# IntelLabs/GKL

Hardware: AMD Instinct MI355X
Metric: pairhmm_gcups (higher is better)
Workload: dtype f32

## Files before the change

### gkl_amd/csrc/pairhmm_aux_kernels.h

```cpp
#pragma once
#include <hip/hip_runtime.h>
#include <stdint.h>

#include "../../include/gkl_hip_pairhmm.h"
#include "pairhmm_fwd_kernel.h"
#include "pairhmm_multi_sets.h"

namespace gklhip {

struct PrepArgs {
  const uint8_t* hap_bases;
  const int32_t* hap_src;
  const int32_t* hap_len;
  const int32_t* hap_pos;
  const int32_t* hap_group;
  const int32_t* hap_pos_flat;
  uint32_t* stream_flat;
  uint32_t* stream;
  uint8_t* hap_has_n;
  int32_t n_haps;
  int32_t* clear_a; int32_t n_a;
  int32_t* clear_b; int32_t n_b;
  int32_t* clear_c; int32_t n_c;
  const uint4* pull_src; uint4* pull_dst; int32_t pull_n16;
// ... 189 lines not shown
  int32_t* count;
  int32_t* read_fail;
  int32_t n_haps;
  int64_t n;
  int mode;
  float log10_init_f;
  double log10_init32_as_f64;
  double log10_init_d;
};

__global__ void finalize32_kernel(FinalizeArgs a) {
  const int64_t i = (int64_t)blockIdx.x * blockDim.x + threadIdx.x;
  if (i >= a.n || a.used64[i]) return;
  const float v = a.raw32[i];
  if (a.mode == GKLHIP_FINALIZE_DEVICE_F64) a.out[i] = log10((double)v) - a.log10_init32_as_f64;
  else if (a.mode == GKLHIP_FINALIZE_DEVICE_REF32) a.out[i] = (double)((float)log10((double)v) - a.log10_init_f);
}

__global__ void finalize64_kernel(FinalizeArgs a, int all_pairs) {
  const int64_t p = (int64_t)blockIdx.x * blockDim.x + threadIdx.x;
  if (p >= a.n) return;
  if (all_pairs) a.used64[p] = 1;
  else if (!a.used64[p]) return;
  if (a.mode >= 0) a.out[p] = log10(a.raw64[p]) - a.log10_init_d;
  if (a.mode == kModePacked) reinterpret_cast<uint64_t*>(a.out)[p] = packed_word(a.raw64[p]);
}

#ifndef GKL_PACK_WINDOW
#define GKL_PACK_WINDOW 96
#endif
constexpr int kPackWindow = GKL_PACK_WINDOW;
constexpr int kJobClasses = 64;
constexpr int kPlanBlock = 1024;

struct PlanArgs {
  FinalizeArgs fa;
  int32_t n_reads, n_haps, n_pairs_i;
  const int64_t* read_off;
  int32_t rpl;
  int32_t max_len;
  int32_t* cnts;
  int32_t* hist;
  int32_t* pos;
  int32_t* order;
  LaneSlot* lanes2;
  const int32_t* hap_orig;
  const int32_t* hap_group;
  const int32_t* hap_pos;
  const int32_t* hap_len;
  FwdJob* jobs;
  FwdJob* sorted;
  const LaneSlot* long_lanes;
  int32_t n_long;
  FwdJob* jobs_long;
  int32_t* long_chunk_jobs;
  int32_t total_cols;
  int32_t wanted_jobs;
  int32_t min_job_cols;
  int32_t packed_by_kernels;
};

__device__ __forceinline__ bool last_block_done(int32_t* arrivals) {
  __shared__ int32_t s_is_last;
  __syncthreads();
  if (threadIdx.x == 0) {
    __threadfence();
    const int32_t before = atomicAdd(arrivals, 1);
    s_is_last = before == (int32_t)gridDim.x - 1 ? 1 : 0;
    __threadfence();
  }
  __syncthreads();
  return s_is_last != 0;
}

__device__ __forceinline__ int32_t ld_cnt(int32_t* p) { return __hip_atomic_load(p, __ATOMIC_RELAXED, __HIP_MEMORY_SCOPE_AGENT); }

__device__ __forceinline__ int job_class(const FwdJob& j, const int32_t* hap_pos, const int32_t* hap_len) {
  const int cols = hap_pos[j.hap_end - 1] + hap_len[j.hap_end - 1] - hap_pos[j.hap_begin];
  const int c = cols >> 7;
  return kJobClasses - 1 - (c < kJobClasses - 1 ? c : kJobClasses - 1);
}

__device__ __forceinline__ void build_jobs_for_chunk(const PlanArgs& a, const LaneSlot* lanes, int c, FwdJob* jobs,
                                                     int32_t* chunk_jobs, int cut_cols, bool by_group, int lane) {
  const LaneSlot sl = lanes[(int64_t)c * kLanes + lane];
  jobs += (int64_t)c * a.n_haps;
  int n_jobs = 0;
  bool prev_need = false;
  uint64_t reads = __ballot(sl.read >= 0 && sl.block == 0);
  for (int k0 = 0; k0 < a.n_haps; k0 += kLanes) {
    const int k = k0 + lane;
    const bool in = k < a.n_haps;
    const int h = in ? a.hap_orig[k] : 0;
    uint8_t nd = 0;
    for (uint64_t m = reads; m; m &= m - 1) {
      const int r = __builtin_amdgcn_readlane(sl.read, __builtin_ctzll(m));
      if (in) nd |= a.fa.used64[(int64_t)r * a.n_haps + h];
    }
    const uint64_t need = __ballot(in && nd != 0);
    if (!need) { prev_need = false; continue; }
    bool start = false;
    if (in && nd) {
      const bool pred_needed = lane == 0 ? prev_need : ((need >> (lane - 1)) & 1ull) != 0;
      start = !pred_needed || a.hap_pos[k - 1] / cut_cols != a.hap_pos[k] / cut_cols ||
              (by_group && a.hap_group[k - 1] != a.hap_group[k]);
    }
    const uint64_t starts = __ballot(start);
    if ((need & 1ull) && !(starts & 1ull)) {
      const uint64_t stop = starts | ~need;
      const int e = stop ? __builtin_ctzll(stop) : kLanes;
      if (lane == 0) jobs[n_jobs - 1].hap_end = min(k0 + e, a.n_haps);
    }
    const int base = n_jobs;
    n_jobs += __builtin_popcountll(starts);
    if (start) {
      const uint64_t after = lane == kLanes - 1 ? 0ull : (~0ull << (lane + 1));
      const uint64_t stop = (starts | ~need) & after;
      const int e = stop ? __builtin_ctzll(stop) : kLanes;
      FwdJob j;
      j.chunk = c; j.hap_begin = k; j.hap_end = min(k0 + e, a.n_haps);
      j.klass = 0;
      jobs[base + __builtin_popcountll(starts & ((1ull << lane) - 1ull))] = j;
    }
    prev_need = ((need >> (kLanes - 1)) & 1ull) != 0;
  }
  __threadfence_block();
  for (int i = lane; i < n_jobs; i += kLanes) {
    FwdJob j = jobs[i];
    jobs[i].klass = job_class(j, a.hap_pos, a.hap_len);
  }
  if (lane == 0) chunk_jobs[c] = n_jobs;
}

#define GKLHIP_PLAN_STAMP(k) do { if (tid == 0) a.cnts[16 + (k)] = (int32_t)(wall_clock64() - clk0); } while (0)

constexpr int kPlanLdsBins = 4096;
template <bool kInLds>
__device__ __forceinline__ void order_affected_reads(const PlanArgs& a, int32_t* hist, int32_t* pos, int32_t* s_wave_tot,
                                                     int tid, uint64_t clk0) {
  constexpr int kBatch = 4;
  const int n = a.n_haps, lane = tid & 63, wave = tid >> 6;
  if (kInLds) {
    for (int c = tid; c < n + 2; c += kPlanBlock) hist[c] = 0;
    __syncthreads();
  }
  for (int r0 = tid; r0 < a.n_reads; r0 += kBatch * kPlanBlock) {
    int f[kBatch];
#pragma unroll
    for (int k = 0; k < kBatch; k++) {
      const int r = r0 + k * kPlanBlock;
      const bool in = r < a.n_reads;
      const int fr = in ? a.fa.read_fail[r] : 0;
      const int64_t len = in ? a.read_off[r + 1] - a.read_off[r] : 0;
      f[k] = (fr > 0 && len <= a.max_len) ? fr : 0;
    }
#pragma unroll
    for (int k = 0; k < kBatch; k++)
      if (f[k] > 0) atomicAdd(hist + f[k], 1);
  }
  __threadfence();
  __syncthreads();
  GKLHIP_PLAN_STAMP(0);

  {
    const int per = (n + kPlanBlock - 1) / kPlanBlock;
    const int hi = n - tid * per, lo = max(hi - per, 0);
    int sum = 0;
    for (int c = hi; c > lo; c--) sum += hist[c];
    int inc = sum;
    for (int d = 1; d < 64; d <<= 1) {
      const int o = __shfl_up(inc, d, 64);
      if (lane >= d) inc += o;
    }
    if (lane == 63) s_wave_tot[wave] = inc;
    __syncthreads();
    int base = 0, total = 0;
    for (int w = 0; w < kPlanBlock / 64; w++) {
      const int t = s_wave_tot[w];
      base += w < wave ? t : 0;
      total += t;
    }
    if (tid == 0) __hip_atomic_store(a.cnts + 4, total, __ATOMIC_RELAXED, __HIP_MEMORY_SCOPE_AGENT);
    int acc = base + inc - sum;
    for (int c = hi; c > lo; c--) { pos[c] = acc; acc += hist[c]; }
  }
  __threadfence();
  __syncthreads();
  GKLHIP_PLAN_STAMP(1);

  for (int r0 = tid; r0 < a.n_reads; r0 += kBatch * kPlanBlock) {
    int f[kBatch];
#pragma unroll
// ... 29 lines not shown
        const int leader = __builtin_ctzll(mask);
        const int32_t read = fails ? (int32_t)((uint32_t)i / (uint32_t)a.n_haps) : -1;
        const int32_t lead_read = __shfl(read, leader, 64);
        const uint64_t same = __ballot(fails && read == lead_read);
        if (lane == leader) atomicAdd(a.fa.read_fail + lead_read, __builtin_popcountll(same));
        if (fails && read != lead_read) atomicAdd(a.fa.read_fail + read, 1);
        if (lane == 0) my_fails += __builtin_popcountll(mask);
      }
      if (in_range) {
        a.fa.used64[i] = fails ? 1 : 0;
        if (a.fa.mode == kModePacked && !a.packed_by_kernels)
          reinterpret_cast<uint64_t*>(a.fa.out)[i] = fails ? 0ull : (kPackedF32Tag | (uint64_t)__float_as_uint(v));
      }
    }
    if (lane == 0) s_wave[wave] = my_fails;
    __syncthreads();
    if (tid == 0) {
      int total = 0;
      for (int w = 0; w < kPlanBlock / 64; w++) total += s_wave[w];
      if (total) atomicAdd(a.cnts + 0, total);
    }
  }
  if (!last_block_done(a.cnts + 10)) return;
  const int n_fail = ld_cnt(a.cnts + 0);
  if (n_fail == 0) return;
  const uint64_t clk0 = wall_clock64();

  if (a.n_haps + 2 <= kPlanLdsBins) order_affected_reads<true>(a, s_hist, s_hist + kPlanLdsBins, s_i32, tid, clk0);
  else                             order_affected_reads<false>(a, a.hist, a.pos, s_i32, tid, clk0);
  GKLHIP_PLAN_STAMP(2);
}

__global__ __launch_bounds__(kPlanBlock) void plan_pack_kernel(PlanArgs a) {
  const int tid = (int)threadIdx.x, lane = tid & 63, wave = tid >> 6;
  const int nblk = (int)gridDim.x, blk = (int)blockIdx.x;
  if (ld_cnt(a.cnts + 0) == 0) return;
  const uint64_t clk0 = wall_clock64();

  {
    static_assert(kPackWindow <= 2 * kLanes, "the window's lane counts sit in two registers per lane");
    __shared__ int32_t s_pack[kPlanBlock / 64][4][kPackWindow];
    int32_t* s_read = s_pack[wave][0]; int32_t* s_needl = s_pack[wave][1]; int32_t* s_sread = s_pack[wave][2];
    int32_t* s_sneed = s_pack[wave][3];
    const int n = ld_cnt(a.cnts + 4);
    const int n_win = (n + kPackWindow - 1) / kPackWindow;
    for (int w = blk * (kPlanBlock / 64) + wave; w < n_win; w += nblk * (kPlanBlock / 64)) {
      const int w0 = w * kPackWindow;
      const int cnt = min(kPackWindow, n - w0);
      for (int i = lane; i < cnt; i += kLanes) {
        const int r = a.order[w0 + i];
        s_read[i] = r;
        s_needl[i] = (int)((a.read_off[r + 1] - a.read_off[r] + a.rpl) / a.rpl);
      }
      __builtin_amdgcn_wave_barrier();
      if (w == 0 && lane == 0) a.cnts[22] = (int32_t)(wall_clock64() - clk0);
      for (int i = lane; i < cnt; i += kLanes) {
        const int ni = s_needl[i];
        int rank = 0;
        for (int j = 0; j < cnt; j++) {
          const int nj = s_needl[j];
          rank += (nj > ni) || (nj == ni && j < i);
        }
        s_sread[rank] = s_read[i];
        s_sneed[rank] = ni;
      }
      __builtin_amdgcn_wave_barrier();
      if (w == 0 && lane == 0) a.cnts[23] = (int32_t)(wall_clock64() - clk0);
      int head = -1, next_lo = -1, next_hi = -1;
      int bin_lo = 0, off_lo = 0, bin_hi = 0, off_hi = 0;
      uint64_t avail = 0;
      int nb = 0;
      const int need_lo = lane < cnt ? s_sneed[lane] : 0, need_hi = lane + kLanes < cnt ? s_sneed[lane + kLanes] : 0;
      for (int i = 0; i < cnt; i++) {
        const int nn = __builtin_amdgcn_readlane(i < kLanes ? need_lo : need_hi, i & 63);
        const uint64_t fits = nn >= kLanes ? 0ull : (avail >> nn) << nn;
        int bin, f;
        if (fits) {
          f = __builtin_ctzll(fits);
          bin = __builtin_amdgcn_readlane(head, f);
          const int nxt = __builtin_amdgcn_readlane(bin < kLanes ? next_lo : next_hi, bin & 63);
          if (lane == f) head = nxt;
          if (nxt < 0) avail &= ~(1ull << f);
        } else {
          bin = nb++;
          f = kLanes;
        }
        const int left = f - nn;
        if (left > 0) {
          const int old = __builtin_amdgcn_readlane(head, left);
          if (lane == (bin & 63)) { if (bin < kLanes) next_lo = old; else next_hi = old; }
          if (lane == left) head = bin;
          avail |= 1ull << left;
        }
        if (lane == (i & 63)) { if (i < kLanes) { bin_lo = bin; off_lo = kLanes - f; } else { bin_hi = bin; off_hi = kLanes - f; } }
      }
      if (w == 0 && lane == 0) a.cnts[24] = (int32_t)(wall_clock64() - clk0);
      int base = 0;
      if (lane == 0) base = atomicAdd(a.cnts + 5, nb);
      base = __shfl(base, 0, kLanes);
      LaneSlot idle; idle.read = -1; idle.block = 0;
      for (int i = lane; i < nb * kLanes; i += kLanes) a.lanes2[(int64_t)base * kLanes + i] = idle;
      __builtin_amdgcn_wave_barrier();
      __threadfence_block();
      if (w == 0 && lane == 0) a.cnts[25] = (int32_t)(wall_clock64() - clk0);
      if (lane < cnt) {
        LaneSlot sl; sl.read = s_sread[lane];
        LaneSlot* dst = a.lanes2 + (int64_t)(base + bin_lo) * kLanes + off_lo;
        for (int b = 0; b < need_lo; b++) { sl.block = b; dst[b] = sl; }
      }
      if (lane + kLanes < cnt) {
        LaneSlot sl; sl.read = s_sread[lane + kLanes];
        LaneSlot* dst = a.lanes2 + (int64_t)(base + bin_hi) * kLanes + off_hi;
        for (int b = 0; b < need_hi; b++) { sl.block = b; dst[b] = sl; }
      }
      __builtin_amdgcn_wave_barrier();
      if (w == 0 && lane == 0) a.cnts[26] = (int32_t)(wall_clock64() - clk0);
    }
  }
  if (blk == 0) GKLHIP_PLAN_STAMP(3);
}

__global__ __launch_bounds__(kPlanBlock) void plan_jobs_kernel(PlanArgs a) {
  __shared__ int32_t s_i32[kPlanBlock];
  const int tid = (int)threadIdx.x, lane = tid & 63, wave = tid >> 6;
  const int nblk = (int)gridDim.x, blk = (int)blockIdx.x;
  const int n_fail = ld_cnt(a.cnts + 0);
  if (n_fail == 0) return;
  const uint64_t clk0 = wall_clock64();

  {
    const int total = ld_cnt(a.cnts + 5);
    const int n_fail_reads = ld_cnt(a.cnts + 4);
    const double density = (double)n_fail / ((double)max(n_fail_reads, 1) * (double)a.n_haps);
    const double est_steps = (double)max(total, 1) * (double)a.total_cols * fmin(density, 1.0);
    const int cut_cols = max(a.min_job_cols, (int)fmin(est_steps / (double)a.wanted_jobs, 1e9));
    const int n_waves = nblk * (kPlanBlock / 64), w = blk * (kPlanBlock / 64) + wave;
    for (int c = w; c < total; c += n_waves) build_jobs_for_chunk(a, a.lanes2, c, a.jobs, a.order, cut_cols, false, lane);
    for (int c = w; c < a.n_long; c += n_waves) build_jobs_for_chunk(a, a.long_lanes, c, a.jobs_long, a.long_chunk_jobs, 0x7fffffff, true, lane);
  }
  if (!last_block_done(a.cnts + 11)) return;
  GKLHIP_PLAN_STAMP(4);

  {
    int32_t* cnt = s_i32;
    int32_t* base = s_i32 + kJobClasses;
    const int total = ld_cnt(a.cnts + 5);
    __syncthreads();
    if (tid < kJobClasses) cnt[tid] = 0;
    __syncthreads();
    for (int c = tid; c < total; c += kPlanBlock) {
      const FwdJob* mine = a.jobs + (int64_t)c * a.n_haps;
      const int n = a.order[c];
      for (int i = 0; i < n; i++) atomicAdd(&cnt[mine[i].klass], 1);
    }
    __syncthreads();
    if (tid == 0) {
      int acc = 0;
      for (int c = 0; c < kJobClasses; c++) { base[c] = acc; acc += cnt[c]; }
      a.cnts[2] = acc;
    }
    __syncthreads();
    for (int c = tid; c < total; c += kPlanBlock) {
      const FwdJob* mine = a.jobs + (int64_t)c * a.n_haps;
      const int n = a.order[c];
      for (int i = 0; i < n; i++) {
        const FwdJob j = mine[i];
        a.sorted[atomicAdd(&base[j.klass], 1)] = j;
      }
    }
    if (tid == 0 && a.n_long > 0) {
      int at = 0;
      for (int c = 0; c < a.n_long; c++) {
        const int n = a.long_chunk_jobs[c];
        for (int i = 0; i < n; i++) a.jobs_long[at++] = a.jobs_long[(int64_t)c * a.n_haps + i];
      }
      a.cnts[8] = at;
    }
  }
  GKLHIP_PLAN_STAMP(5);
}
#undef GKLHIP_PLAN_STAMP

__global__ void flush_selftest_kernel(uint32_t* out, float f, double d) {
  float fm;
  double dm;
  asm volatile("v_mul_f32 %0, 1.0, %1" : "=v"(fm) : "v"(f));
  asm volatile("v_mul_f64 %0, 1.0, %1" : "=v"(dm) : "v"(d));
  out[0] = __float_as_uint(fm);
  out[1] = (uint32_t)((uint64_t)__double_as_longlong(dm) >> 32) | (uint32_t)(uint64_t)__double_as_longlong(dm);
}

__global__ __launch_bounds__(256) void lds_oob_selftest_kernel(uint32_t* out) {
  __shared__ __attribute__((aligned(16))) uint32_t lds[4 * 2560];
  for (int i = threadIdx.x; i < 4 * 2560; i += 256) lds[i] = 0xA5A50000u | (uint32_t)i;
  __syncthreads();
  const uint32_t loff = (uint32_t)(uintptr_t)lds + (threadIdx.x >> 6) * 10240u + (threadIdx.x & 63u) * 16u;
  uint32_t acc = 0;
#pragma unroll
  for (int shift = 9; shift <= 11; shift++) {
    const uint32_t addr = (512u << shift) + loff;
    uint32_t v0, v1, v2, v3, w0, w1, w2, w3, x0, x1;
    asm volatile("ds_read_b128 v[40:43], %10\n\tds_read_b128 v[44:47], %10 offset:1024\n\tds_read_b64 v[48:49], %10\n\ts_waitcnt lgkmcnt(0)\n\t"
                 "v_mov_b32 %0, v40\n\tv_mov_b32 %1, v41\n\tv_mov_b32 %2, v42\n\tv_mov_b32 %3, v43\n\t"
                 "v_mov_b32 %4, v44\n\tv_mov_b32 %5, v45\n\tv_mov_b32 %6, v46\n\tv_mov_b32 %7, v47\n\tv_mov_b32 %8, v48\n\tv_mov_b32 %9, v49"
                 : "=v"(v0), "=v"(v1), "=v"(v2), "=v"(v3), "=v"(w0), "=v"(w1), "=v"(w2), "=v"(w3), "=v"(x0), "=v"(x1)
                 : "v"(addr) : "v40", "v41", "v42", "v43", "v44", "v45", "v46", "v47", "v48", "v49", "memory");
    acc |= v0 | v1 | v2 | v3 | w0 | w1 | w2 | w3 | x0 | x1;
// ... 198 lines not shown
```

### gkl_amd/csrc/pairhmm_device_pass.h

```cpp
#pragma once

namespace {

int aux_streams(DevCtx* c) {
  if (!c->upload_stream) HIP_TRY(hipStreamCreateWithFlags(&c->upload_stream, hipStreamNonBlocking));
  if (!c->copy_stream) {
    HIP_TRY(hipStreamCreateWithFlags(&c->copy_stream, hipStreamNonBlocking));
    if (!c->pad_stream) HIP_TRY(hipStreamCreateWithFlags(&c->pad_stream, hipStreamNonBlocking));
  }
  return GKLHIP_OK;
}

template <typename T>
int upload_tables(DevCtx* c, const HostTables<T>& h, DevBuf* buf, DevTables<T>* dt) {
  const size_t n = (size_t)kQuals * 2 + kMmEntries;
  int st = buf->reserve(n * sizeof(T));
  if (st) return st;
  T* base = buf->as<T>();
  {
    T* pin = nullptr;
    HIP_TRY(hipHostMalloc(reinterpret_cast<void**>(&pin), n * sizeof(T), hipHostMallocDefault));
    memcpy(pin, h.ph2pr.data(), kQuals * sizeof(T));
    memcpy(pin + kQuals, h.div3.data(), kQuals * sizeof(T));
    memcpy(pin + 2 * kQuals, h.mm.data(), kMmEntries * sizeof(T));
// ... 112 lines not shown
    return;
  }
  const int waves = std::max(2, std::min(kWideWavesMax, (blocks_for(max_read_len, RPL) + kLanes - 1) / kLanes));
  if (fma) {
    if (waves == 2)      hipLaunchKernelGGL((pairhmm_fwd_wide_kernel<T, RPL, true, 2>), dim3(n_blocks), dim3(128), 0, s, a, carry, carry_len);
    else if (waves == 3) hipLaunchKernelGGL((pairhmm_fwd_wide_kernel<T, RPL, true, 3>), dim3(n_blocks), dim3(192), 0, s, a, carry, carry_len);
    else                 hipLaunchKernelGGL((pairhmm_fwd_wide_kernel<T, RPL, true, 4>), dim3(n_blocks), dim3(256), 0, s, a, carry, carry_len);
  } else {
    if (waves == 2)      hipLaunchKernelGGL((pairhmm_fwd_wide_kernel<T, RPL, false, 2>), dim3(n_blocks), dim3(128), 0, s, a, carry, carry_len);
    else if (waves == 3) hipLaunchKernelGGL((pairhmm_fwd_wide_kernel<T, RPL, false, 3>), dim3(n_blocks), dim3(192), 0, s, a, carry, carry_len);
    else                 hipLaunchKernelGGL((pairhmm_fwd_wide_kernel<T, RPL, false, 4>), dim3(n_blocks), dim3(256), 0, s, a, carry, carry_len);
  }
}

struct SmallLaunch {
  SmallCall call;
  const SmallCall* desc_pinned = nullptr;
  const SmallCall* desc_dev = nullptr;
};

#ifndef GKL_RPL_F64
#define GKL_RPL_F64 6
#endif
constexpr int kRplF64 = GKL_RPL_F64;
#ifndef GKL_RPL_F64_JOBS
#define GKL_RPL_F64_JOBS 10
#endif
constexpr int kRplF64Jobs = GKL_RPL_F64_JOBS;
constexpr int kRplF64Wide = 8;
constexpr size_t kSmallBatchBytes = 1 << 20;
constexpr int64_t kDirectPairs = 65536;
constexpr int64_t kTwoStepFrom = 2048;
constexpr int64_t kSmallDoublePairs = kTwoStepFrom;
constexpr int kPlanBlocks = 64;
constexpr int kFallbackWantedJobs = 12288;
constexpr int64_t kHostShardPairs = 400000;
constexpr int64_t kOnePassPairs = 65536;
constexpr int kTargetCols = 2048;
#ifndef GKL_RPL_F32
#define GKL_RPL_F32 8
#endif
constexpr int kRplF32 = GKL_RPL_F32;
std::atomic<int> g_host_calls_in_flight{0};
int pick_f32_rpl(int forced, int n_reads, int n_haps, const int64_t* read_off, const int64_t* hap_off, int load = 1) {
  int max_len = 0;
  for (int r = 0; r < n_reads; r++) max_len = std::max(max_len, (int)(read_off[r + 1] - read_off[r]));
  if (forced == 2 && max_len <= 2 * kLanes - 1) return 2;
  if (forced == 4 || forced == -4 || forced == 2) return 4;
  if (forced == 8) return kRplF32;
  const int64_t total_cols = hap_off[n_haps] + n_haps;
  auto jobs_at = [&](int rpl) {
    int64_t blocks = 0;
    for (int r = 0; r < n_reads; r++) {
      const int nb = blocks_for((int)(read_off[r + 1] - read_off[r]), rpl);
      if (nb <= kLanes) blocks += nb;
    }
    const int64_t chunks = std::max<int64_t>(1, (blocks + kLanes - 1) / kLanes);
    const int64_t groups = std::min<int64_t>(n_haps, std::max<int64_t>((total_cols + kTargetCols - 1) / kTargetCols,
                                                                        (4096 + chunks - 1) / chunks));
    return chunks * groups;
  };
  if (jobs_at(kRplF32) * load >= 2048 || max_len > 4 * kLanes - 1) return kRplF32;
  if (jobs_at(4) * load >= 1024 || max_len > 2 * kLanes - 1) return 4;
  return 2;
}

void launch_main_f32(const FwdArgs<float>& a, int rpl_main, int fma, int n_blocks, hipStream_t s) {
// ... 264 lines not shown
  int rc;
  const int slot = c->plan_slot ^= 1;
  PinBuf& stage = c->stage_slot[slot];
  DevBuf& plan_dev = c->plan_dev_slot[slot];
  HIP_TRY(hipEventSynchronize(c->stage_free_slot[slot]));
  if (L.total > stage.cap || L.total > plan_dev.cap) HIP_TRY(hipEventSynchronize(c->plan_unused_slot[slot]));
  if ((rc = stage.reserve(L.total))) return rc;
  if ((rc = plan_dev.reserve(L.total))) return rc;
  unsigned char* hs = stage.as<unsigned char>();
  fill_plan_block(hs, P, plan, c->long_lanes, c->long_jobs, db);
  unsigned char* dp = plan_dev.as<unsigned char>();
  if (c->have_call_done && c->last_stream != s) HIP_TRY(hipStreamWaitEvent(s, c->call_done, 0));
  S.hs_dev = nullptr;
  if (P.pull) {
    void* p = nullptr;
    HIP_TRY(hipHostGetDevicePointer(&p, hs, 0));
    S.hs_dev = static_cast<const unsigned char*>(p);
    if (!P.defers) HIP_TRY(hipStreamWaitEvent(s, c->plan_unused_slot[slot], 0));
  } else {
    if ((rc = aux_streams(c))) return rc;
    HIP_TRY(hipStreamWaitEvent(c->upload_stream, c->plan_unused_slot[slot], 0));
    HIP_TRY(hipMemcpyAsync(dp, hs, L.total, hipMemcpyHostToDevice, c->upload_stream));
    HIP_TRY(hipEventRecord(c->stage_free_slot[slot], c->upload_stream));
    HIP_TRY(hipStreamWaitEvent(s, c->stage_free_slot[slot], 0));
  }
  if (g_env.timing)
    fprintf(stderr, "[gklhip] host plan + staging: %.3f ms (%d chunks, %d stream entries, %zu plan bytes)\n",
            std::chrono::duration<double, std::milli>(std::chrono::steady_clock::now() - P.t0).count(),
            plan.n_chunks, plan.n_stream, L.total);

  if ((rc = c->raw32.reserve((size_t)P.n_pairs * 4))) return rc;
  if ((rc = c->raw64.reserve((size_t)P.n_pairs * 8))) return rc;
  if ((rc = c->used64.reserve((size_t)P.n_pairs))) return rc;
  if ((rc = c->counters.reserve(128))) return rc;
  if ((rc = c->read_fail.reserve((size_t)P.n_reads * 4))) return rc;
  if ((rc = c->stream_buf.reserve(((size_t)plan.n_stream + (size_t)plan.n_stream_flat) * 4))) return rc;
  if (!P.use_double && (rc = c->fail_hist.reserve((size_t)P.n_hist * 4))) return rc;
  if ((rc = c->hap_flags.reserve((size_t)P.n_haps))) return rc;
  if ((rc = c->lanes_main.reserve((size_t)std::max(plan.n_chunks, 1) * kLanes * sizeof(LaneSlot)))) return rc;

  S.s = s; S.out = out_dev; S.slot = slot; S.hs = hs; S.dp = dp; S.xcarry = nullptr;
  const gklhip_batch dbi = P.inline_host ? batch_at(*db, dp + L.batch, L.batch_stride) : *db;
  S.b = DevBatch{dbi.read_bases, dbi.read_quals, dbi.ins_gop, dbi.del_gop, dbi.gcp, reinterpret_cast<const int64_t*>(dp + L.read_off), P.n_reads, P.n_haps};
  S.hap_bases = (P.pull && P.inline_host) ? batch_at(*db, S.hs_dev + L.batch, L.batch_stride).hap_bases : dbi.hap_bases;
  S.stream_grouped = P.inline_host ? reinterpret_cast<uint32_t*>(dp + L.stream) : c->stream_buf.as<uint32_t>();
  S.stream_flat = P.inline_host ? reinterpret_cast<uint32_t*>(dp + L.stream_flat) : c->stream_buf.as<uint32_t>() + plan.n_stream;
  S.hap_has_n = P.inline_host ? dp + L.has_n : c->hap_flags.as<uint8_t>();
  return GKLHIP_OK;
}

PrepArgs prep_args(const DevCtx* c, const CallPlan& P, const StagedCall& S) {
  const PlanLayout& L = P.L;
  PrepArgs pa;
  const unsigned char* pb = P.pull ? S.hs_dev : S.dp;
  pa.hap_bases = S.hap_bases;
  pa.hap_src = reinterpret_cast<const int32_t*>(pb + L.hap_src);
  pa.hap_len = reinterpret_cast<const int32_t*>(pb + L.hap_len);
  pa.hap_pos = reinterpret_cast<const int32_t*>(pb + L.hap_pos);
  pa.hap_group = reinterpret_cast<const int32_t*>(pb + L.hap_group);
  pa.stream = S.stream_grouped;
  pa.hap_pos_flat = P.use_double ? nullptr : reinterpret_cast<const int32_t*>(pb + L.hap_pos_flat);
  pa.stream_flat = S.stream_flat;
  pa.hap_has_n = S.hap_has_n;
  pa.n_haps = P.inline_host ? 0 : P.n_haps;
  pa.clear_a = c->counters.as<int32_t>(); pa.n_a = 32;
  pa.clear_b = c->read_fail.as<int32_t>(); pa.n_b = P.use_double ? 0 : P.n_reads;
  pa.clear_c = c->fail_hist.as<int32_t>(); pa.n_c = P.n_hist;
  pa.place_chunk = reinterpret_cast<const int32_t*>(pb + L.place_chunk);
  pa.place_lane = pb + L.place_lane;
  pa.chunk_used = pb + L.chunk_used;
  pa.read_off = reinterpret_cast<const int64_t*>(pb + L.read_off);
  pa.lanes_out = c->lanes_main.as<LaneSlot>();
  pa.n_reads = P.n_reads; pa.n_chunks = c->plan.n_chunks; pa.rpl = P.rpl_main;
  const int threads_needed = std::max({pa.n_haps * 64, 32, pa.n_b, pa.n_c, P.n_reads});
  pa.hap_blocks = (threads_needed + kPrepBlock - 1) / kPrepBlock;
  pa.pull_src = reinterpret_cast<const uint4*>(S.hs_dev);
  pa.pull_dst = reinterpret_cast<uint4*>(S.dp);
  pa.pull_n16 = P.pull ? (int32_t)(L.total / 16) : 0;
  return pa;
}
int prep_grid(const PrepArgs& pa, const CallPlan& P) {
  return pa.hap_blocks + (P.pull ? (int)std::min<size_t>(64, (P.L.total / 16 + kPrepBlock * 4 - 1) / (kPrepBlock * 4)) : 0);
}

template <typename T>
FwdArgs<T> fwd_args(const DevCtx* c, const CallPlan& P, const StagedCall& S) {
  constexpr bool is_f32 = std::is_same<T, float>::value;
  const PlanLayout& L = P.L;
  unsigned char* dp = S.dp;
  FwdArgs<T> a{};
  a.b = S.b;
  a.stream = S.stream_grouped;
  a.hap_len = reinterpret_cast<const int32_t*>(dp + L.hap_len);
  a.hap_pos = reinterpret_cast<const int32_t*>(dp + L.hap_pos);
  a.hap_orig = reinterpret_cast<const int32_t*>(dp + L.hap_orig);
  a.hap_has_n = S.hap_has_n;
  a.groups = reinterpret_cast<const HapGroup*>(dp + L.groups);
  a.n_groups = (int)c->plan.groups.size();
  a.chunk_lanes = c->lanes_main.as<LaneSlot>();
  a.n_chunks = c->plan.n_chunks;
  a.chunk_stride = P.chunk_stride;
  a.jobs = c->jobs.as<FwdJob>();
  a.job_count = c->counters.as<int32_t>() + 2;
  a.job_next = c->counters.as<int32_t>() + 3;
  a.asm_general = (c->asm_general && (!is_f32 || c->lds_oob_zero)) ? 1 : 0;
  if constexpr (is_f32) {
    a.tab = c->dt32;
// ... 31 lines not shown
  fa.count = c->counters.as<int32_t>(); fa.n = P.n_pairs; fa.mode = P.finalize_mode;
  fa.read_fail = c->read_fail.as<int32_t>(); fa.n_haps = P.n_haps;
  fa.log10_init_f = host_tables_f32().log10_initial; fa.log10_init32_as_f64 = std::log10(std::ldexp(1.0, 120)); fa.log10_init_d = host_tables_f64().log10_initial;
  return fa;
}
PairPolicyArgs pair_policy_args(const DevCtx* c, const CallPlan& P, const StagedCall& S) {
  PairPolicyArgs q;
  q.raw32 = c->raw32.as<float>(); q.out = S.out; q.used64 = c->used64.as<uint8_t>(); q.count = c->counters.as<int32_t>();
  q.hap_sidx = reinterpret_cast<const int32_t*>(S.dp + P.L.hap_sidx);
  q.mode = P.finalize_mode;
  q.log10_init_f = host_tables_f32().log10_initial; q.log10_init32_as_f64 = std::log10(std::ldexp(1.0, 120)); q.log10_init_d = host_tables_f64().log10_initial;
  return q;
}
size_t planned_max_jobs(const CallPlan& P) { return (size_t)P.n_reads * (size_t)P.n_haps; }
PlanArgs plan_args(const DevCtx* c, const CallPlan& P, const StagedCall& S) {
  const PlanLayout& L = P.L;
  unsigned char* dp = S.dp;
  const int n_reads = P.n_reads, n_haps = P.n_haps;
  PlanArgs pa;
  pa.fa = finalize_args(c, P, S);
  pa.n_reads = n_reads; pa.n_haps = n_haps; pa.n_pairs_i = (int32_t)P.n_pairs;
  pa.read_off = S.b.read_off;
  pa.rpl = kRplF64Jobs; pa.max_len = kLanes * kRplF64Jobs - 1;
  pa.cnts = c->counters.as<int32_t>();
  pa.hist = c->fail_hist.as<int32_t>();
  pa.pos = pa.hist + (n_haps + 2);
  pa.order = c->fail_order.as<int32_t>();
  pa.lanes2 = c->lanes2.as<LaneSlot>();
  pa.hap_orig = reinterpret_cast<const int32_t*>(dp + L.hap_orig);
  pa.hap_group = reinterpret_cast<const int32_t*>(dp + L.hap_group);
  pa.hap_pos = reinterpret_cast<const int32_t*>(dp + L.hap_pos_flat);
  pa.hap_len = reinterpret_cast<const int32_t*>(dp + L.hap_len);
  pa.jobs = c->jobs.as<FwdJob>();
  pa.sorted = c->jobs.as<FwdJob>() + planned_max_jobs(P);
  pa.long_lanes = reinterpret_cast<const LaneSlot*>(dp + L.long_lanes) + (size_t)P.n_long_main * kLanes;
  pa.n_long = P.n_long64;
  pa.jobs_long = c->jobs_long.as<FwdJob>();
  pa.long_chunk_jobs = c->fail_order.as<int32_t>() + n_reads;
  pa.total_cols = (int32_t)std::min<int64_t>((int64_t)P.hl + n_haps, 0x7fffffff);
  pa.wanted_jobs = g_env.fb_wanted_jobs > 0 ? g_env.fb_wanted_jobs : (int)std::min<int64_t>(kFallbackWantedJobs, std::max<int64_t>(4096, P.n_pairs / 100));
  pa.min_job_cols = 256;
  pa.packed_by_kernels = (P.finalize_mode == kModePacked && !P.per_pair) ? 1 : 0;
  return pa;
}

int launch_prep(DevCtx* c, const CallPlan& P, const StagedCall& S) {
  const bool ev = c->cfg.record_events != 0;
  if (ev) {
    const bool deferred = c->cfg.record_events == 2;
    c->ev = c->ev_ring[deferred ? c->calls % DevCtx::kEventRing : 0];
    c->ring_double[deferred ? c->calls % DevCtx::kEventRing : 0] = P.use_double;
    c->calls++;
    HIP_TRY(hipEventRecord(c->ev[0], S.s));
  }
  const PrepArgs pa = prep_args(c, P, S);
  hipLaunchKernelGGL(prep_kernel, dim3((unsigned)prep_grid(pa, P)), dim3(kPrepBlock), 0, S.s, pa);
  if (P.pull) HIP_TRY(hipEventRecord(c->stage_free_slot[S.slot], S.s));
  return GKLHIP_OK;
}
int reserve_carry(DevCtx* c, const CallPlan& P, StagedCall* S) {
  if (P.n_long_main == 0 && P.n_long64 == 0) return GKLHIP_OK;
  if (int rc = c->carry.reserve(P.striped_carry_bytes + (size_t)super_blocks_max<float>() * 2 * (size_t)P.xsteps * 32)) return rc;
  if (P.xsteps > 0) S->xcarry = c->carry.as<unsigned char>() + P.striped_carry_bytes;
  return GKLHIP_OK;
}
int launch_all_double(DevCtx* c, const CallPlan& P, const StagedCall& S) {
  const bool ev = c->cfg.record_events != 0;
// ... 17 lines not shown
    if (P.rpl_main <= 4) launch_long<float, 4>(la, P.fma, P.n_long_waves, c->carry.as<float>(), P.carry_len, s);
    else                 launch_long_jobs<float, kRplF32, kRplF32>(la, P.fma, P.n_long_waves, c->plan.max_read_len, c->carry.as<float>(), P.carry_len, s, S.xcarry, P.xsteps, c->counters.as<int32_t>() + 12);
  }
  if (c->cfg.record_events != 0) HIP_TRY(hipEventRecord(c->ev[2], s));
  return GKLHIP_OK;
}
int launch_per_pair(DevCtx* c, const CallPlan& P, const StagedCall& S, const FwdArgs<float>& a) {
  const bool ev = c->cfg.record_events != 0;
  hipStream_t s = S.s;
  const FwdArgs<double> d = recompute_args(c, P, S);
  const PairPolicyArgs q = pair_policy_args(c, P, S);
  if (ev) HIP_TRY(hipEventRecord(c->ev[3], s));
  if (P.fused) {
    if (int rc = launch_pair_fused(a, d, q, P.rows, P.fma, P.n_pairs, s, c->speculate_fp64 && g_host_calls_in_flight.load(std::memory_order_relaxed) <= 1)) return rc;
  } else if (P.n_pairs > kTwoStepFrom) {
    if (int rc = c->fail_order.reserve((size_t)P.n_pairs * 4)) return rc;
    if (int rc = launch_pair_policy_two_step(d, q, P.rows, P.fma, P.n_pairs, c->fail_order.as<int32_t>(), s)) return rc;
  } else {
    if (int rc = launch_pair_policy(d, q, P.rows, P.fma, P.n_pairs, s)) return rc;
  }
  if (ev) HIP_TRY(hipEventRecord(c->ev[4], s));
  HIP_TRY(hipEventRecord(c->policy_done, s));
  return GKLHIP_OK;
}
int launch_planned_fp64(DevCtx* c, const CallPlan& P, const StagedCall& S) {
  const bool ev = c->cfg.record_events != 0;
  hipStream_t s = S.s;
  const int n_reads = P.n_reads;
  const int64_t n_pairs = P.n_pairs;
  const size_t max_jobs = planned_max_jobs(P);
  int rc;
  if ((rc = c->fail_order.reserve(((size_t)n_reads + (size_t)P.n_long64) * 4))) return rc;
  if ((rc = c->lanes2.reserve((size_t)n_reads * kLanes * sizeof(LaneSlot)))) return rc;
  if ((rc = c->jobs.reserve(2 * max_jobs * sizeof(FwdJob)))) return rc;
  if (P.n_long64 > 0 && (rc = c->jobs_long.reserve((size_t)P.n_long64 * (size_t)P.n_haps * sizeof(FwdJob)))) return rc;
  const PlanArgs pa = plan_args(c, P, S);
  const int blocks_env = g_env.plan_blocks;
  const int policy_grid = std::max(1, blocks_env > 0 ? blocks_env : (int)std::min<int64_t>(c->n_cus, std::max<int64_t>(16, n_pairs / 4096)));
  const int64_t max_windows = ((int64_t)n_reads + kPackWindow - 1) / kPackWindow;
  const int pack_grid = (int)std::max<int64_t>(1, std::min<int64_t>(kPlanBlocks, (max_windows + kPlanBlock / 64 - 1) / (kPlanBlock / 64)));
  const int jobs_grid = std::max(1, std::min(c->n_cus, blocks_env > 0 ? blocks_env : (int)std::min<int64_t>(kPlanBlocks, std::max<int64_t>(16, n_pairs / 8192))));
  hipLaunchKernelGGL(plan_policy_kernel, dim3((unsigned)policy_grid), dim3(kPlanBlock), 0, s, pa);
  HIP_TRY(hipEventRecord(c->policy_done, s));
  hipLaunchKernelGGL(plan_pack_kernel, dim3((unsigned)pack_grid), dim3(kPlanBlock), 0, s, pa);
  hipLaunchKernelGGL(plan_jobs_kernel, dim3((unsigned)jobs_grid), dim3(kPlanBlock), 0, s, pa);
  const bool side_finalize = finalizes_on_device(P.finalize_mode);
  if (side_finalize) {
    if ((rc = aux_streams(c))) return rc;
    HIP_TRY(hipStreamWaitEvent(c->copy_stream, c->policy_done, 0));
    hipLaunchKernelGGL(finalize32_kernel, dim3((unsigned)((n_pairs + 255) / 256)), dim3(256), 0, c->copy_stream, pa.fa);
    HIP_TRY(hipEventRecord(c->early_copy_done, c->copy_stream));
  }
  FwdArgs<double> d = recompute_args(c, P, S);
  d.chunk_lanes = c->lanes2.as<LaneSlot>();
  d.n_chunks = n_reads;
  d.jobs = c->jobs.as<FwdJob>() + max_jobs;
  if (ev) HIP_TRY(hipEventRecord(c->ev[3], s));
  launch_jobs<double, kRplF64Jobs>(d, P.fma, (int)std::min<int64_t>(n_pairs, (int64_t)c->n_cus * 16), s);
  if (P.n_long64 > 0) {
    int32_t* cnts = c->counters.as<int32_t>();
    FwdArgs<double> ld = d;
    ld.chunk_lanes = pa.long_lanes;
    ld.jobs = c->jobs_long.as<FwdJob>();
    ld.job_count = cnts + 8;
    ld.job_next = cnts + 9;
    launch_long_jobs<double, kRplF64Wide, kRplF64>(ld, P.fma, P.n_long_waves, c->plan.max_read_len, c->carry.as<double>(), P.carry_len, s, S.xcarry, P.xsteps, cnts + 13);
  }
  if (ev) HIP_TRY(hipEventRecord(c->ev[4], s));
  hipLaunchKernelGGL(finalize64_kernel, dim3((unsigned)((n_pairs + 255) / 256)), dim3(256), 0, s, pa.fa, 0);
  if (side_finalize) HIP_TRY(hipStreamWaitEvent(s, c->early_copy_done, 0));
  return GKLHIP_OK;
}
int finish_call(DevCtx* c, const CallPlan& P, const StagedCall& S) {
  const bool ev = c->cfg.record_events != 0;
  hipStream_t s = S.s;
  gklhip_stats& st = c->stats;
  if (ev) HIP_TRY(hipEventRecord(c->ev[5], s));
  HIP_TRY(hipGetLastError());
// ... 89 lines not shown
```

Baseline: 4748.

## Fuse job building into pack kernel with per-window class counting and dense scatter

Merges plan_jobs_kernel into plan_pack_kernel. Each block now handles one window: it rank-sorts the reads using all waves, packs them with wave 0, then builds jobs for that window's chunks right away. Per-class job counts are gathered in LDS and reserved with global atomics into a dense array, so the last block only scatters dense jobs by class instead of serially walking every chunk's job list. The cut size comes from a lane estimate counted during the policy pass, and the grid limit goes up. This removes a kernel launch and the serial single-block sort, at the cost of more scratch memory, more atomics, and a cut_cols based on an estimate.

```diff
diff --git a/gkl_amd/csrc/pairhmm_aux_kernels.h b/gkl_amd/csrc/pairhmm_aux_kernels.h
--- a/gkl_amd/csrc/pairhmm_aux_kernels.h
+++ b/gkl_amd/csrc/pairhmm_aux_kernels.h
@@ -245,6 +245,8 @@
 constexpr int kPackWindow = GKL_PACK_WINDOW;
 constexpr int kJobClasses = 64;
 constexpr int kPlanBlock = 1024;
+constexpr int kPlanCounters = 32 + kJobClasses;
+constexpr int kPackLanesFilled = 62;
 
 struct PlanArgs {
   FinalizeArgs fa;
@@ -262,6 +264,8 @@
   const int32_t* hap_pos;
   const int32_t* hap_len;
   FwdJob* jobs;
+  FwdJob* dense;
+  uint8_t* dense_class;
   FwdJob* sorted;
   const LaneSlot* long_lanes;
   int32_t n_long;
@@ -294,7 +298,7 @@
   return kJobClasses - 1 - (c < kJobClasses - 1 ? c : kJobClasses - 1);
 }
 
-__device__ __forceinline__ void build_jobs_for_chunk(const PlanArgs& a, const LaneSlot* lanes, int c, FwdJob* jobs,
+__device__ __forceinline__ int build_jobs_for_chunk(const PlanArgs& a, const LaneSlot* lanes, int c, FwdJob* jobs,
                                                      int32_t* chunk_jobs, int cut_cols, bool by_group, int lane) {
   const LaneSlot sl = lanes[(int64_t)c * kLanes + lane];
   jobs += (int64_t)c * a.n_haps;
@@ -338,11 +342,8 @@
     prev_need = ((need >> (kLanes - 1)) & 1ull) != 0;
   }
   __threadfence_block();
-  for (int i = lane; i < n_jobs; i += kLanes) {
-    FwdJob j = jobs[i];
-    jobs[i].klass = job_class(j, a.hap_pos, a.hap_len);
-  }
-  if (lane == 0) chunk_jobs[c] = n_jobs;
+  if (chunk_jobs && lane == 0) chunk_jobs[c] = n_jobs;
+  return n_jobs;
 }
 
 #define GKLHIP_PLAN_STAMP(k) do { if (tid == 0) a.cnts[16 + (k)] = (int32_t)(wall_clock64() - clk0); } while (0)
@@ -357,6 +358,7 @@
     for (int c = tid; c < n + 2; c += kPlanBlock) hist[c] = 0;
     __syncthreads();
   }
+  int lanes_needed = 0;
   for (int r0 = tid; r0 < a.n_reads; r0 += kBatch * kPlanBlock) {
     int f[kBatch];
 #pragma unroll
@@ -366,11 +368,14 @@
       const int fr = in ? a.fa.read_fail[r] : 0;
       const int64_t len = in ? a.read_off[r + 1] - a.read_off[r] : 0;
       f[k] = (fr > 0 && len <= a.max_len) ? fr : 0;
+      if (f[k] > 0) lanes_needed += (int)((len + a.rpl) / a.rpl);
     }
 #pragma unroll
     for (int k = 0; k < kBatch; k++)
       if (f[k] > 0) atomicAdd(hist + f[k], 1);
   }
+  for (int d = 32; d > 0; d >>= 1) lanes_needed += __shfl_down(lanes_needed, d, 64);
+  if (lane == 0 && lanes_needed > 0) atomicAdd(a.cnts + 14, lanes_needed);
   __threadfence();
   __syncthreads();
   GKLHIP_PLAN_STAMP(0);
@@ -466,40 +471,61 @@
 }
 
 __global__ __launch_bounds__(kPlanBlock) void plan_pack_kernel(PlanArgs a) {
+  __shared__ int32_t s_i32[kJobClasses];
+  __shared__ int32_t s_pack[4][kPackWindow];
+  __shared__ int32_t s_chunks[2];
+  __shared__ int32_t s_class[kJobClasses + 1];
+  __shared__ int32_t s_first[kPackWindow], s_count[kPackWindow];
   const int tid = (int)threadIdx.x, lane = tid & 63, wave = tid >> 6;
   const int nblk = (int)gridDim.x, blk = (int)blockIdx.x;
-  if (ld_cnt(a.cnts + 0) == 0) return;
+  const int n_fail = ld_cnt(a.cnts + 0);
+  if (n_fail == 0) return;
   const uint64_t clk0 = wall_clock64();
-
-  {
+  const int n = ld_cnt(a.cnts + 4);
+  const int n_win = (n + kPackWindow - 1) / kPackWindow;
+  const int est_chunks = (ld_cnt(a.cnts + 14) + kPackLanesFilled - 1) / kPackLanesFilled;
+  const double density = (double)n_fail / ((double)max(n, 1) * (double)a.n_haps);
+  const double est_steps = (double)max(est_chunks, 1) * (double)a.total_cols * fmin(density, 1.0);
+  const int cut_cols = max(a.min_job_cols, (int)fmin(est_steps / (double)a.wanted_jobs, 1e9));
+
+  for (int w = blk; w < n_win; w += nblk) {
+    if (tid <= kJobClasses) s_class[tid] = 0;
     static_assert(kPackWindow <= 2 * kLanes, "the window's lane counts sit in two registers per lane");
-    __shared__ int32_t s_pack[kPlanBlock / 64][4][kPackWindow];
-    int32_t* s_read = s_pack[wave][0]; int32_t* s_needl = s_pack[wave][1]; int32_t* s_sread = s_pack[wave][2];
-    int32_t* s_sneed = s_pack[wave][3];
-    const int n = ld_cnt(a.cnts + 4);
-    const int n_win = (n + kPackWindow - 1) / kPackWindow;
-    for (int w = blk * (kPlanBlock / 64) + wave; w < n_win; w += nblk * (kPlanBlock / 64)) {
-      const int w0 = w * kPackWindow;
-      const int cnt = min(kPackWindow, n - w0);
-      for (int i = lane; i < cnt; i += kLanes) {
-        const int r = a.order[w0 + i];
-        s_read[i] = r;
-        s_needl[i] = (int)((a.read_off[r + 1] - a.read_off[r] + a.rpl) / a.rpl);
+    static_assert(kPlanBlock == 8 * 2 * kLanes, "rank sort: eight threads per read of a window");
+    int32_t* s_read = s_pack[0]; int32_t* s_needl = s_pack[1]; int32_t* s_sread = s_pack[2];
+    int32_t* s_sneed = s_pack[3];
+    int32_t* s_rank = s_first;
+    const int w0 = w * kPackWindow;
+    const int cnt = min(kPackWindow, n - w0);
+    if (tid < cnt) {
+      const int r = a.order[w0 + tid];
+      s_read[tid] = r;
+      s_needl[tid] = (int)((a.read_off[r + 1] - a.read_off[r] + a.rpl) / a.rpl);
+      s_rank[tid] = 0;
+    }
+    __syncthreads();
+    if (w == 0 && tid == 0) a.cnts[22] = (int32_t)(wall_clock64() - clk0);
+    {
+      const int i = tid & (2 * kLanes - 1);
+      if (i < cnt) {
+        const int ni = s_needl[i];
+        int before = 0;
+        for (int j = tid >> 7; j < cnt; j += 8) {
+          const int nj = s_needl[j];
+          before += (nj > ni) || (nj == ni && j < i);
+        }
+        if (before) atomicAdd(&s_rank[i], before);
       }
-      __builtin_amdgcn_wave_barrier();
-      if (w == 0 && lane == 0) a.cnts[22] = (int32_t)(wall_clock64() - clk0);
-      for (int i = lane; i < cnt; i += kLanes) {
-        const int ni = s_needl[i];
-        int rank = 0;
-        for (int j = 0; j < cnt; j++) {
-          const int nj = s_needl[j];
-          rank += (nj > ni) || (nj == ni && j < i);
-        }
-        s_sread[rank] = s_read[i];
-        s_sneed[rank] = ni;
-      }
-      __builtin_amdgcn_wave_barrier();
-      if (w == 0 && lane == 0) a.cnts[23] = (int32_t)(wall_clock64() - clk0);
+    }
+    __syncthreads();
+    if (tid < cnt) {
+      const int rank = s_rank[tid];
+      s_sread[rank] = s_read[tid];
+      s_sneed[rank] = s_needl[tid];
+    }
+    __syncthreads();
+    if (w == 0 && tid == 0) a.cnts[23] = (int32_t)(wall_clock64() - clk0);
+    if (wave == 0) {
       int head = -1, next_lo = -1, next_hi = -1;
       int bin_lo = 0, off_lo = 0, bin_hi = 0, off_hi = 0;
       uint64_t avail = 0;
@@ -549,64 +575,75 @@
       }
       __builtin_amdgcn_wave_barrier();
       if (w == 0 && lane == 0) a.cnts[26] = (int32_t)(wall_clock64() - clk0);
-    }
-  }
-  if (blk == 0) GKLHIP_PLAN_STAMP(3);
-}
-
-__global__ __launch_bounds__(kPlanBlock) void plan_jobs_kernel(PlanArgs a) {
-  __shared__ int32_t s_i32[kPlanBlock];
-  const int tid = (int)threadIdx.x, lane = tid & 63, wave = tid >> 6;
-  const int nblk = (int)gridDim.x, blk = (int)blockIdx.x;
-  const int n_fail = ld_cnt(a.cnts + 0);
-  if (n_fail == 0) return;
-  const uint64_t clk0 = wall_clock64();
-
-  {
-    const int total = ld_cnt(a.cnts + 5);
-    const int n_fail_reads = ld_cnt(a.cnts + 4);
-    const double density = (double)n_fail / ((double)max(n_fail_reads, 1) * (double)a.n_haps);
-    const double est_steps = (double)max(total, 1) * (double)a.total_cols * fmin(density, 1.0);
-    const int cut_cols = max(a.min_job_cols, (int)fmin(est_steps / (double)a.wanted_jobs, 1e9));
-    const int n_waves = nblk * (kPlanBlock / 64), w = blk * (kPlanBlock / 64) + wave;
-    for (int c = w; c < total; c += n_waves) build_jobs_for_chunk(a, a.lanes2, c, a.jobs, a.order, cut_cols, false, lane);
-    for (int c = w; c < a.n_long; c += n_waves) build_jobs_for_chunk(a, a.long_lanes, c, a.jobs_long, a.long_chunk_jobs, 0x7fffffff, true, lane);
-  }
+      if (lane == 0) { s_chunks[0] = base; s_chunks[1] = nb; }
+    }
+    __syncthreads();
+    if (w == 0) GKLHIP_PLAN_STAMP(3);
+    const int c0 = s_chunks[0], c1 = c0 + s_chunks[1];
+    for (int c = c0 + wave; c < c1; c += kPlanBlock / 64) {
+      const int n_jobs = build_jobs_for_chunk(a, a.lanes2, c, a.jobs, nullptr, cut_cols, false, lane);
+      FwdJob* mine = a.jobs + (int64_t)c * a.n_haps;
+      for (int i = lane; i < n_jobs; i += kLanes) mine[i].klass = atomicAdd(&s_class[job_class(mine[i], a.hap_pos, a.hap_len)], 1);
+      if (lane == 0) { s_first[c - c0] = atomicAdd(&s_class[kJobClasses], n_jobs); s_count[c - c0] = n_jobs; }
+    }
+    __syncthreads();
+    if (tid <= kJobClasses) {
+      const int n_mine = s_class[tid];
+      s_class[tid] = n_mine > 0 ? atomicAdd(a.cnts + (tid < kJobClasses ? 32 + tid : 6), n_mine) : 0;
+    }
+    __syncthreads();
+    for (int c = c0 + wave; c < c1; c += kPlanBlock / 64) {
+      const FwdJob* mine = a.jobs + (int64_t)c * a.n_haps;
+      const int n_jobs = s_count[c - c0], first = s_class[kJobClasses] + s_first[c - c0];
+      for (int i = lane; i < n_jobs; i += kLanes) {
+        FwdJob j = mine[i];
+        const int k = job_class(j, a.hap_pos, a.hap_len);
+        j.klass += s_class[k];
+        a.dense[first + i] = j;
+        a.dense_class[first + i] = (uint8_t)k;
+      }
+    }
+    __syncthreads();
+  }
+  for (int c = blk * (kPlanBlock / 64) + wave; c < a.n_long; c += nblk * (kPlanBlock / 64))
+    build_jobs_for_chunk(a, a.long_lanes, c, a.jobs_long, a.long_chunk_jobs, 0x7fffffff, true, lane);
   if (!last_block_done(a.cnts + 11)) return;
   GKLHIP_PLAN_STAMP(4);
 
   {
-    int32_t* cnt = s_i32;
-    int32_t* base = s_i32 + kJobClasses;
-    const int total = ld_cnt(a.cnts + 5);
-    __syncthreads();
-    if (tid < kJobClasses) cnt[tid] = 0;
-    __syncthreads();
-    for (int c = tid; c < total; c += kPlanBlock) {
-      const FwdJob* mine = a.jobs + (int64_t)c * a.n_haps;
-      const int n = a.order[c];
-      for (int i = 0; i < n; i++) atomicAdd(&cnt[mine[i].klass], 1);
-    }
+    int32_t* start = s_i32;
+    const int total = ld_cnt(a.cnts + 6);
+    if (tid < kJobClasses) start[tid] = ld_cnt(a.cnts + 32 + tid);
     __syncthreads();
     if (tid == 0) {
       int acc = 0;
-      for (int c = 0; c < kJobClasses; c++) { base[c] = acc; acc += cnt[c]; }
+      for (int c = 0; c < kJobClasses; c++) { const int n_c = start[c]; start[c] = acc; acc += n_c; }
       a.cnts[2] = acc;
     }
     __syncthreads();
-    for (int c = tid; c < total; c += kPlanBlock) {
-      const FwdJob* mine = a.jobs + (int64_t)c * a.n_haps;
-      const int n = a.order[c];
-      for (int i = 0; i < n; i++) {
-        const FwdJob j = mine[i];
-        a.sorted[atomicAdd(&base[j.klass], 1)] = j;
+    constexpr int kBatch = 4;
+    for (int i0 = tid; i0 < total; i0 += kBatch * kPlanBlock) {
+      FwdJob j[kBatch];
+      int k[kBatch];
+#pragma unroll
+      for (int b = 0; b < kBatch; b++) {
+        const int i = min(i0 + b * kPlanBlock, total - 1);
+        j[b] = a.dense[i];
+        k[b] = a.dense_class[i];
       }
+#pragma unroll
+      for (int b = 0; b < kBatch; b++)
+        if (i0 + b * kPlanBlock < total) {
+          const int at = start[k[b]] + j[b].klass;
+          j[b].klass = k[b];
+          a.sorted[at] = j[b];
+        }
     }
     if (tid == 0 && a.n_long > 0) {
       int at = 0;
       for (int c = 0; c < a.n_long; c++) {
-        const int n = a.long_chunk_jobs[c];
-        for (int i = 0; i < n; i++) a.jobs_long[at++] = a.jobs_long[(int64_t)c * a.n_haps + i];
+        const int n_c = a.long_chunk_jobs[c];
+        for (int i = 0; i < n_c; i++) a.jobs_long[at++] = a.jobs_long[(int64_t)c * a.n_haps + i];
       }
       a.cnts[8] = at;
     }
diff --git a/gkl_amd/csrc/pairhmm_device_pass.h b/gkl_amd/csrc/pairhmm_device_pass.h
--- a/gkl_amd/csrc/pairhmm_device_pass.h
+++ b/gkl_amd/csrc/pairhmm_device_pass.h
@@ -168,7 +168,7 @@
 constexpr int64_t kDirectPairs = 65536;
 constexpr int64_t kTwoStepFrom = 2048;
 constexpr int64_t kSmallDoublePairs = kTwoStepFrom;
-constexpr int kPlanBlocks = 64;
+constexpr int kPlanBlocks = 256;
 constexpr int kFallbackWantedJobs = 12288;
 constexpr int64_t kHostShardPairs = 400000;
 constexpr int64_t kOnePassPairs = 65536;
@@ -499,7 +499,7 @@
   if ((rc = c->raw32.reserve((size_t)P.n_pairs * 4))) return rc;
   if ((rc = c->raw64.reserve((size_t)P.n_pairs * 8))) return rc;
   if ((rc = c->used64.reserve((size_t)P.n_pairs))) return rc;
-  if ((rc = c->counters.reserve(128))) return rc;
+  if ((rc = c->counters.reserve(kPlanCounters * 4))) return rc;
   if ((rc = c->read_fail.reserve((size_t)P.n_reads * 4))) return rc;
   if ((rc = c->stream_buf.reserve(((size_t)plan.n_stream + (size_t)plan.n_stream_flat) * 4))) return rc;
   if (!P.use_double && (rc = c->fail_hist.reserve((size_t)P.n_hist * 4))) return rc;
@@ -530,7 +530,7 @@
   pa.stream_flat = S.stream_flat;
   pa.hap_has_n = S.hap_has_n;
   pa.n_haps = P.inline_host ? 0 : P.n_haps;
-  pa.clear_a = c->counters.as<int32_t>(); pa.n_a = 32;
+  pa.clear_a = c->counters.as<int32_t>(); pa.n_a = kPlanCounters;
   pa.clear_b = c->read_fail.as<int32_t>(); pa.n_b = P.use_double ? 0 : P.n_reads;
   pa.clear_c = c->fail_hist.as<int32_t>(); pa.n_c = P.n_hist;
   pa.place_chunk = reinterpret_cast<const int32_t*>(pb + L.place_chunk);
@@ -539,7 +539,7 @@
   pa.read_off = reinterpret_cast<const int64_t*>(pb + L.read_off);
   pa.lanes_out = c->lanes_main.as<LaneSlot>();
   pa.n_reads = P.n_reads; pa.n_chunks = c->plan.n_chunks; pa.rpl = P.rpl_main;
-  const int threads_needed = std::max({pa.n_haps * 64, 32, pa.n_b, pa.n_c, P.n_reads});
+  const int threads_needed = std::max({pa.n_haps * 64, kPlanCounters, pa.n_b, pa.n_c, P.n_reads});
   pa.hap_blocks = (threads_needed + kPrepBlock - 1) / kPrepBlock;
   pa.pull_src = reinterpret_cast<const uint4*>(S.hs_dev);
   pa.pull_dst = reinterpret_cast<uint4*>(S.dp);
@@ -637,7 +637,9 @@
   pa.hap_pos = reinterpret_cast<const int32_t*>(dp + L.hap_pos_flat);
   pa.hap_len = reinterpret_cast<const int32_t*>(dp + L.hap_len);
   pa.jobs = c->jobs.as<FwdJob>();
-  pa.sorted = c->jobs.as<FwdJob>() + planned_max_jobs(P);
+  pa.sorted = pa.jobs + planned_max_jobs(P);
+  pa.dense = pa.sorted + planned_max_jobs(P);
+  pa.dense_class = reinterpret_cast<uint8_t*>(pa.dense + planned_max_jobs(P));
   pa.long_lanes = reinterpret_cast<const LaneSlot*>(dp + L.long_lanes) + (size_t)P.n_long_main * kLanes;
   pa.n_long = P.n_long64;
   pa.jobs_long = c->jobs_long.as<FwdJob>();
@@ -721,18 +723,16 @@
   int rc;
   if ((rc = c->fail_order.reserve(((size_t)n_reads + (size_t)P.n_long64) * 4))) return rc;
   if ((rc = c->lanes2.reserve((size_t)n_reads * kLanes * sizeof(LaneSlot)))) return rc;
-  if ((rc = c->jobs.reserve(2 * max_jobs * sizeof(FwdJob)))) return rc;
+  if ((rc = c->jobs.reserve(3 * max_jobs * sizeof(FwdJob) + max_jobs))) return rc;
   if (P.n_long64 > 0 && (rc = c->jobs_long.reserve((size_t)P.n_long64 * (size_t)P.n_haps * sizeof(FwdJob)))) return rc;
   const PlanArgs pa = plan_args(c, P, S);
   const int blocks_env = g_env.plan_blocks;
   const int policy_grid = std::max(1, blocks_env > 0 ? blocks_env : (int)std::min<int64_t>(c->n_cus, std::max<int64_t>(16, n_pairs / 4096)));
   const int64_t max_windows = ((int64_t)n_reads + kPackWindow - 1) / kPackWindow;
-  const int pack_grid = (int)std::max<int64_t>(1, std::min<int64_t>(kPlanBlocks, (max_windows + kPlanBlock / 64 - 1) / (kPlanBlock / 64)));
-  const int jobs_grid = std::max(1, std::min(c->n_cus, blocks_env > 0 ? blocks_env : (int)std::min<int64_t>(kPlanBlocks, std::max<int64_t>(16, n_pairs / 8192))));
+  const int pack_grid = (int)std::max<int64_t>(1, std::min<int64_t>(blocks_env > 0 ? blocks_env : kPlanBlocks, max_windows));
   hipLaunchKernelGGL(plan_policy_kernel, dim3((unsigned)policy_grid), dim3(kPlanBlock), 0, s, pa);
   HIP_TRY(hipEventRecord(c->policy_done, s));
   hipLaunchKernelGGL(plan_pack_kernel, dim3((unsigned)pack_grid), dim3(kPlanBlock), 0, s, pa);
-  hipLaunchKernelGGL(plan_jobs_kernel, dim3((unsigned)jobs_grid), dim3(kPlanBlock), 0, s, pa);
   const bool side_finalize = finalizes_on_device(P.finalize_mode);
   if (side_finalize) {
     if ((rc = aux_streams(c))) return rc;
```

Result: no change. 4769 (median of 6 runs) (+0.5%).
